# uci-cbcl/RP-Net

Measured on AMD Instinct MI355X. Metric: support/query pairs/sec (fwd+bwd, 1-shot 256x256, T=5), higher is better.
Workload: dtype f32

## Files before the change

rpnet_amd/csrc/conv_split.hip:

```cpp
#include <algorithm>

#include "conv_epilogue.h"
#include "split_bf16.h"

namespace rpnet {

constexpr bool IGLP = true;

template <int NP>
__global__ __launch_bounds__(256) void split_bf16_kernel(const float* __restrict__ x, const float* __restrict__ scale,
                                                          const int mode, unsigned short* __restrict__ out,
                                                          const size_t n8, const FastDiv fC, const size_t plane_elems) {
    RPNET_PASS_PRIORITY();
    for (size_t i = (size_t)blockIdx.x * 256 + threadIdx.x; i < n8; i += (size_t)gridDim.x * 256) {
        const f32x4 a = *reinterpret_cast<const f32x4*>(x + i * 8);
        const f32x4 b = *reinterpret_cast<const f32x4*>(x + i * 8 + 4);
        float v[8] = {a[0], a[1], a[2], a[3], b[0], b[1], b[2], b[3]};
        if (mode) {
            float s = scale[fC.div((unsigned)i)];
            if (mode == 2) s = 1.f - s;
#pragma unroll
            for (int q = 0; q < 8; ++q) v[q] *= s;
        }
        u32x4 o[NP];
        split8<NP>(v, o);
#pragma unroll
        for (int p = 0; p < NP; ++p) *reinterpret_cast<u32x4*>(out + p * plane_elems + i * 8) = o[p];
    }
}

template <int NP>
__global__ __launch_bounds__(256) void split_f16_kernel(const float* __restrict__ x, const float* __restrict__ mask, const int mode,
                                                         const float* __restrict__ s_a, const float* __restrict__ s_b,
                                                         float* __restrict__ s_out, unsigned short* __restrict__ out,
                                                         const size_t n8, const FastDiv fC, const size_t plane_elems,
// ... 137 lines not shown
                if (NP <= 2) {
                    const float inv = 1.f / u_row[row];
#pragma unroll
                    for (int q = 0; q < 8; ++q) v[q] *= inv;
                }
                u32x4 o[NP];
                split8<NP>(v, o);
                const int tf = taps - 1 - tap;
                const size_t dst = (((size_t)tf * (Cout >> 5) + (co0 >> 5)) * Cin_g + row) * 32 + g * 8;
#pragma unroll
                for (int p = 0; p < NP; ++p) *reinterpret_cast<u32x4*>(wd + p * plane + dst) = o[p];
            }
        }
    }
}

__host__ __device__ static inline bool pack_needs_gather(const rpnet_pack_item& q) {
    return (q.cin % 8) || (q.cin_off0 % 8) || (q.cin_split % 8) || (q.cin_off1 % 8);
}

template <int NP>
__global__ __launch_bounds__(256) void pack_weight_split_kernel(const PackItems items) {
    __shared__ float tile[9][32][33];
    const rpnet_pack_item& q = items.it[blockIdx.y];
    const bool gather = pack_needs_gather(q);
    const int tx = gather ? q.cin_pad / 32 : (q.cin + 31) / 32, ntiles = tx * (q.cout / 32);
    if ((int)blockIdx.x >= ntiles) return;
    if (gather)
        pack_weight_split_block<NP, true>(tile, blockIdx.x % tx, blockIdx.x / tx, q.w, (unsigned short*)q.wp, (unsigned short*)q.wd, q.taps,
                                          q.cin_pad, q.cout, q.cin, q.cin_off0, q.cin_split, q.cin_off1, q.row_scale_wp, q.row_scale_wd);
    else
        pack_weight_split_block<NP, false>(tile, blockIdx.x % tx, blockIdx.x / tx, q.w, (unsigned short*)q.wp, (unsigned short*)q.wd, q.taps,
                                           q.cin_pad, q.cout, q.cin, q.cin_off0, q.cin_split, q.cin_off1, q.row_scale_wp, q.row_scale_wd);
}

template <int WGM, int WM, int WN, int NP, bool DB>
__global__ __launch_bounds__(WGM * 128, (DB ? 1 : (WGM == 2 ? 2 : 1))) void conv_igemm_split_kernel(
    const rpnet_conv_desc d, const int M, const int Cin, const int Cout, const int tiles_n, const int ntiles) {
    constexpr int NT = WGM * 128;
    constexpr int BM = 32 * WGM * WM, BN = 64 * WN;
    constexpr int RP = NT / 4;
    constexpr int AJ = BM / RP, BJ = (BN + RP - 1) / RP;
    constexpr bool B_PART = BN < RP;
    constexpr int A_BYTES = BM * 64, B_BYTES = BN * 64;
    constexpr int STAGE = NP * (A_BYTES + B_BYTES);
    __shared__ __attribute__((aligned(16))) unsigned char smem[cmax((DB ? 2 : 1) * STAGE, epilogue_lds_bytes<WN, WGM>())];

    const int t = threadIdx.x;
    const int lane = t & 63, wv = t >> 6;
    const int li = lane & 31, h = lane >> 5;
    const int wm = wv >> 1, wn = wv & 1;

    const int tile = xcd_swizzle(blockIdx.x, ntiles);
    const int tm = tile / tiles_n, tn = tile - tm * tiles_n;
    const int m0 = tm * BM, n0 = tn * BN;

    const int H = d.H, W = d.W, HW = H * W;
    const int ups = d.upsample;
    const int Hs = H >> ups, Ws = W >> ups;
    const int dil = d.dilation > 1 ? d.dilation : 1;

    const int srow = t >> 2, skg = t & 3;
    int rn[AJ], ry[AJ], rx[AJ];
#pragma unroll
    for (int j = 0; j < AJ; ++j) {
        const int m = m0 + srow + RP * j;
// ... 783 lines not shown
    using namespace rpnet;
    RPNET_REQUIRE(items && n >= 1 && n <= kPackMax, RPNET_ERR_ARG, "pack_conv_weights_split: %d items (1..%d)", n, kPackMax);
    RPNET_REQUIRE(planes >= 1 && planes <= 3, RPNET_ERR_SHAPE, "pack_conv_weights_split: planes %d", planes);
    PackItems pk;
    int max_rows = 0, max_tiles = 0;
    for (int i = 0; i < n; ++i) {
        const rpnet_pack_item& q = items[i];
        RPNET_REQUIRE(q.w && q.wp, RPNET_ERR_ARG, "pack_conv_weights_split: null pointer (item %d)", i);
        RPNET_REQUIRE(planes == 3 || (q.row_scale_wp && q.row_scale_wd), RPNET_ERR_ARG,
                      "pack_conv_weights_split: fp16 planes (1 or 2) need the row scale outputs (item %d)", i);
        RPNET_REQUIRE(q.cout > 0 && q.cout % 32 == 0 && q.cin_pad % 32 == 0 && (q.taps == 9 || q.taps == 1 || q.taps == 4), RPNET_ERR_SHAPE,
                      "pack_conv_weights_split: cout %d cin_pad %d taps %d (item %d)", q.cout, q.cin_pad, q.taps, i);
        RPNET_REQUIRE(q.cin > 0 && q.cin_split >= 0 && q.cin_split <= q.cin && q.cin_off0 >= 0 && q.cin_off1 >= 0, RPNET_ERR_SHAPE,
                      "pack_conv_weights_split: cin %d cin_split %d cin_off0 %d cin_off1 %d (item %d)", q.cin, q.cin_split, q.cin_off0,
                      q.cin_off1, i);
        RPNET_REQUIRE((long)q.cin_off0 + q.cin_split <= q.cin_pad && (long)q.cin_off1 + (q.cin - q.cin_split) <= q.cin_pad, RPNET_ERR_SHAPE,
                      "pack_conv_weights_split: channel ranges exceed cin_pad (item %d)", i);
        RPNET_REQUIRE(pack_ranges_disjoint(q.cin, q.cin_off0, q.cin_split, q.cin_off1), RPNET_ERR_SHAPE,
                      "pack_conv_weights_split: channel ranges overlap (item %d)", i);
        pk.it[i] = q;
        max_rows = std::max(max_rows, q.cout + q.cin);
        max_tiles = std::max(max_tiles, (pack_needs_gather(q) ? q.cin_pad / 32 : cdiv(q.cin, 32)) * (q.cout / 32));
    }
    for (int i = n; i < kPackMax; ++i) pk.it[i] = items[0];
    hipStream_t s = (hipStream_t)stream;
    if (planes <= 2)
        hipLaunchKernelGGL(weight_row_scale_kernel, dim3(max_rows, n), dim3(256), 0, s, pk);
    if (planes == 3) hipLaunchKernelGGL(pack_weight_split_kernel<3>, dim3(max_tiles, n), dim3(256), 0, s, pk);
    else if (planes == 2) hipLaunchKernelGGL(pack_weight_split_kernel<2>, dim3(max_tiles, n), dim3(256), 0, s, pk);
    else hipLaunchKernelGGL(pack_weight_split_kernel<1>, dim3(max_tiles, n), dim3(256), 0, s, pk);
    return check_launch("pack_conv_weights_split");
}

extern "C" int rpnet_pack_conv_weight_split(const float* w, void* wp, void* wd, int cout, int cin, int taps, int cin_off0,
                                            int cin_split, int cin_off1, int cin_pad, int planes, float* row_scale_wp,
                                            float* row_scale_wd, rpnet_stream_t stream) {
    rpnet_pack_item q;
    q.w = w; q.wp = wp; q.wd = wd; q.row_scale_wp = row_scale_wp; q.row_scale_wd = row_scale_wd;
    q.cout = cout; q.cin = cin; q.taps = taps; q.cin_off0 = cin_off0; q.cin_split = cin_split; q.cin_off1 = cin_off1; q.cin_pad = cin_pad;
    return rpnet_pack_conv_weights_split(&q, 1, planes, stream);
}
```

rpnet_amd/functional.py:

```python
import collections
import contextlib
import ctypes as C
import os

import torch
from torch.autograd import Function
from torch.autograd.function import once_differentiable

from . import hip
from .hip import ConvDesc, call, ptr, query

BN_EPS = 1e-5
BN_MOMENTUM = 0.1

_ASYNC = {"on": False, "side": {}, "pending": set(), "queued": False, "fifo": [], "keep": []}

_MODES = {"f32": (0, False, 0), "bf16x3": (3, False, 0), "f16x2": (3, True, 2), "f16": (3, True, 1)}
_CORR_PRED_PLANES = True
_MATH = {}


def set_conv_math(mode):
    _MATH["mode"] = mode
    _MATH["planes"], _MATH["f16"], _MATH["f16_planes"] = _MODES[mode]
# ... 474 lines not shown
             self.split, self.off1, self.cin_pad)

    @property
    def wp(self):
        if self._wp is None:
            self._pack_f32()
        return self._wp

    @property
    def wd(self):
        if self._wp is None:
            self._pack_f32()
        return self._wd

    def split_packs(self, planes):
        pk = self.wps.get(planes) if self.wps else None
        if pk is None:
            w = self._weight
            pk = self.alloc_split(planes)
            call("rpnet_pack_conv_weight_split", ptr(w), ptr(pk[0]), ptr(pk[1]), self.cout, self.cin, self.taps,
                 self.off0, self.split, self.off1, self.cin_pad, planes, ptr(pk[2]) if planes <= 2 else None,
                 ptr(pk[3]) if planes <= 2 else None)
        return pk

    def up4_packs(self, planes):
        up = getattr(self, "_up4", None)
        if up is None:
            up = self._up4 = {}
        pk = up.get(planes)
        if pk is None:
            w = self._weight
            wc = torch.empty((4 * self.cout, self.cin, 2, 2), device=w.device, dtype=torch.float32)
            call("rpnet_upconv_collapse_weights", ptr(w), ptr(wc), self.cout, self.cin)
            n = 4 * self.cin * 4 * self.cout
            wp4 = torch.empty((planes, n), device=w.device, dtype=torch.float16)
            wd4 = torch.empty((planes, n), device=w.device, dtype=torch.float16)
            t4 = torch.empty(4 * self.cout, device=w.device, dtype=torch.float32)
            u4 = torch.empty(self.cin, device=w.device, dtype=torch.float32)
            call("rpnet_pack_conv_weight_split", ptr(wc), ptr(wp4), ptr(wd4), 4 * self.cout, self.cin, 4, 0, self.cin, self.cin, self.cin,
                 planes, ptr(t4), ptr(u4))
            pk = up[planes] = (wp4, wd4, t4, u4)
        return pk

    def alloc_split(self, planes):
        if self.wps is None:
            self.wps = {}
        n = self.taps * self.cin_pad * self.cout
        padded = self.cin_pad != self.cin
        w = self._weight
        key = (w.data_ptr(), tuple(w.shape), planes, self.cin_pad, self.off0, self.split, self.off1, str(w.device))
        if padded and self._pool is not None and key in self._pool:
            pk = self._pool[key]
            self.wps[planes] = pk
            return pk
        mk = torch.zeros if padded else torch.empty
        dt = torch.bfloat16 if planes == 3 else torch.float16
        wps, wds = mk((planes, n), device=w.device, dtype=dt), mk((planes, n), device=w.device, dtype=dt)
        if planes == 3:
            pk = (wps, wds)
        else:
            t = torch.empty(self.cout, device=w.device, dtype=torch.float32)
            u = (torch.ones if padded else torch.empty)(self.cin_pad, device=w.device, dtype=torch.float32)
            pk = (wps, wds, t, u)
        if padded and self._pool is not None:
            self._pool[key] = pk
        self.wps[planes] = pk
        return pk


class WeightCache:

    def __init__(self):
        self._d = {}
        self._ready = None
        self._padded = {}

    def clear(self):
        self._d.clear()
        self._ready = None

    def prepack_async(self, weights, planes, device, up4=()):
        main = torch.cuda.current_stream(device)
        ps = _pack_stream(device)
        ps.wait_stream(main)
        self._ready = None
        with torch.cuda.stream(ps):
            self.prepack(weights, planes, up4)
            ev = torch.cuda.Event()
            ev.record(ps)
        self._ready = (ev, set(), torch.cuda.is_current_stream_capturing())

    def get(self, weight, split=None):
        if self._ready is not None and self._ready[2] and not torch.cuda.is_current_stream_capturing():
            self._ready = None
        if self._ready is not None:
            sid = hip.stream()
            if sid not in self._ready[1]:
                torch.cuda.current_stream(weight.device).wait_event(self._ready[0])
                self._ready[1].add(sid)
        key = (weight.data_ptr(), weight._version, None if split is None else tuple(split))
        pw = self._d.get(key)
        if pw is None:
            pw = PackedWeight(weight.detach(), split, self._padded)
            self._d[key] = pw
        return pw

    def prepack(self, weights, planes, up4=()):
        up4 = list(up4) if (_UP4 and planes in (1, 2)) else []
        if up4:
            skip = {id(w) for w in up4}
            weights = [w for w in weights if id(w) not in skip]
            for w in up4:
                self.get(w).up4_packs(planes)
        pws = [self.get(w) for w in weights]
        pws = [pw for pw in pws if pw.taps == 9 and pw.cin_pad == pw.cin and pw.cin % 32 == 0 and pw.cout % 32 == 0
               and not (pw.wps and planes in pw.wps)]
        for i in range(0, len(pws), hip.PACK_MAX):
            chunk = pws[i:i + hip.PACK_MAX]
            items = (hip.PackItem * len(chunk))()
            for it, pw in zip(items, chunk):
                bufs = pw.alloc_split(planes)
                it.w, it.wp, it.wd = ptr(pw._weight), ptr(bufs[0]), ptr(bufs[1])
                it.row_scale_wp, it.row_scale_wd = (ptr(bufs[2]), ptr(bufs[3])) if planes <= 2 else (None, None)
                it.cout, it.cin, it.taps = pw.cout, pw.cin, pw.taps
                it.cin_off0, it.cin_split, it.cin_off1, it.cin_pad = pw.off0, pw.split, pw.off1, pw.cin_pad
            call("rpnet_pack_conv_weights_split", items, len(chunk), planes)

    def materialize(self, weights, planes):
        for w in weights:
            pw = self.get(w)
            if planes and pw.taps == 9 and pw.cin_pad == pw.cin and pw.cin % 32 == 0 and pw.cout % 32 == 0:
                pw.split_packs(planes)
            else:
                pw.wp


TUNE = {"tile": int(os.environ.get("RPNET_TUNE_TILE", "0")) + (0 if os.environ.get("RPNET_CONV_DMA", "1") == "1" else 0x10000),
        "wgrad": int(os.environ.get("RPNET_TUNE_WGRAD", "0"))}


def _desc(x0, x1, w, bias, in_scale, in_mode, y0, y1, N, H, W, taps, ups, groups=1, ep_scale=None, ep_shift=None,
          ep_relu=0, out_scale=None, out_mode=0, accumulate=0, co_split=None, wgrad=False):
    d = ConvDesc()
    d.x0, d.x1 = ptr(x0), ptr(x1)
    d.C0 = x0.shape[-1]
    d.C1 = x1.shape[-1] if x1 is not None else 0
    d.w, d.bias = ptr(w), ptr(bias)
    d.in_scale, d.in_scale_mode = ptr(in_scale), in_mode if in_scale is not None else 0
    d.y0, d.y1 = ptr(y0), ptr(y1)
    d.Co0 = y0.shape[-1] if co_split is None else co_split[0]
    d.Co1 = (y1.shape[-1] if y1 is not None else 0) if co_split is None else co_split[1]
    d.ep_scale, d.ep_shift, d.ep_relu = ptr(ep_scale), ptr(ep_shift), ep_relu
    d.out_scale, d.out_scale_mode, d.accumulate = ptr(out_scale), out_mode if out_scale is not None else 0, accumulate
    d.N, d.H, d.W, d.taps, d.upsample, d.groups = N, H, W, taps, ups, groups
    d.tune = TUNE["wgrad"] if wgrad else TUNE["tile"]
    return d


_Plan = collections.namedtuple("_Plan", "kind planes xs w sx sx1 col", defaults=(None, None, None))


def _conv_plan(pw, op0, op1, in_scale, in_mode, upsample, N, H, W, cout, up4_allowed=True):
    x0, x1 = op0.x, None if op1 is None else op1.x
    if not _use_split(pw, x0, x1):
        return _Plan("f32", 0, (x0, x1), pw.wp)
    f16 = _f16_sources(op0, op1, in_scale, in_mode, pw.taps == 1) if f16_mode() else None
    if f16 is None:
# ... 1065 lines not shown
```

rpnet_amd/hip.py:

```python
import ctypes as C
import os

import torch

_LIB_PATH = os.environ.get("RPNET_LIB_PATH") or os.path.join(os.path.dirname(os.path.abspath(__file__)), "librpnet_hip.so")
_lib = None

vp, ci, cf, cs, cd = C.c_void_p, C.c_int, C.c_float, C.c_size_t, C.c_double


class ConvDesc(C.Structure):
    _fields_ = [("x0", vp), ("x1", vp), ("C0", ci), ("C1", ci), ("w", vp), ("bias", vp), ("in_scale", vp),
                ("in_scale_mode", ci), ("y0", vp), ("y1", vp), ("Co0", ci), ("Co1", ci), ("ep_scale", vp),
                ("ep_shift", vp), ("ep_relu", ci), ("out_scale", vp), ("out_scale_mode", ci), ("accumulate", ci),
                ("N", ci), ("H", ci), ("W", ci), ("taps", ci), ("upsample", ci), ("groups", ci), ("dilation", ci), ("stats_partial", vp), ("split_planes", ci), ("y_split", vp), ("split_out_planes", ci),
                ("acc_scale_col", vp), ("acc_scale_x", vp), ("acc_scale_dy", vp), ("bnb_y", vp), ("bnb_stats", vp), ("bnb_partial", vp), ("bnb_pmax", vp), ("bnb_groups", ci),
                ("acc_scale_x1", vp), ("out_absmax", vp), ("tune", ci), ("y_split_scale", vp), ("splitk_ws", vp), ("splitk_ws_bytes", cs),
                ("skip_mask", vp), ("skip_mode", ci), ("skip_halo", ci), ("skip_ws", vp), ("tile_skip", vp),
                ("y_enc", vp), ("y_enc_stride", ci)]


PACK_MAX = 24


class PackItem(C.Structure):
    _fields_ = [("w", vp), ("wp", vp), ("wd", vp), ("row_scale_wp", vp), ("row_scale_wd", vp), ("cout", ci), ("cin", ci),
                ("taps", ci), ("cin_off0", ci), ("cin_split", ci), ("cin_off1", ci), ("cin_pad", ci)]


_SIGS = {
    "rpnet_version": (ci, []),
    "rpnet_last_error_string": (C.c_char_p, []),
    "rpnet_pack_conv_weight": (ci, [vp, vp, vp, ci, ci, ci, ci, ci, ci, ci, vp]),
    "rpnet_split_bf16": (ci, [vp, vp, ci, vp, cs, ci, ci, vp]),
    "rpnet_split_f16": (ci, [vp, vp, ci, vp, vp, vp, vp, cs, ci, ci, ci, vp]),
    "rpnet_pack_conv_weight_split": (ci, [vp, vp, vp, ci, ci, ci, ci, ci, ci, ci, ci, vp, vp, vp]),
    "rpnet_pack_conv_weights_split": (ci, [C.POINTER(PackItem), ci, ci, vp]),
    "rpnet_conv_fwd": (ci, [C.POINTER(ConvDesc), vp]),
    "rpnet_upconv_collapse_weights": (ci, [vp, vp, ci, ci, vp]),
    "rpnet_conv_up4_supported": (ci, [C.POINTER(ConvDesc), ci]),
    "rpnet_conv_up4_stats_blocks": (ci, [C.POINTER(ConvDesc)]),
    "rpnet_conv_up4": (ci, [C.POINTER(ConvDesc), ci, vp]),
    "rpnet_conv_wgrad_up4_supported": (ci, [C.POINTER(ConvDesc)]),
    "rpnet_conv_wgrad_up4_workspace_bytes": (cs, [ci, ci, ci, ci, ci]),
    "rpnet_conv_wgrad_up4": (ci, [C.POINTER(ConvDesc), vp, vp, vp, cs, vp]),
    "rpnet_conv_stats_blocks": (ci, [C.POINTER(ConvDesc)]),
    "rpnet_conv_tile_variant": (ci, [C.POINTER(ConvDesc)]),
    "rpnet_conv_splitk_workspace_bytes": (cs, [C.POINTER(ConvDesc)]),
    "rpnet_bn_stats_from_partial": (ci, [vp, ci, ci, ci, ci, ci, vp, vp, vp, vp, vp, cf, cf, vp, vp, vp, vp, vp]),
    "rpnet_conv_wgrad_workspace_bytes": (cs, [ci, ci, ci, ci, ci, ci]),
    "rpnet_conv_wgrad": (ci, [C.POINTER(ConvDesc), vp, vp, ci, ci, ci, ci, vp, cs, vp]),
    "rpnet_conv1_fwd": (ci, [vp, vp, vp, vp, vp, vp, ci, ci, ci, ci, vp, vp, ci, vp]),
    "rpnet_conv1_stats_blocks": (ci, [ci, ci, ci, ci, ci]),
    "rpnet_pow2_scale": (ci, [vp, vp, vp]),
    "rpnet_predict_scales": (ci, [vp, vp, vp, ci, cf, ci, vp, vp]),
# ... 204 lines not shown
}
VOLLOAD_ABI_SYMBOLS = tuple(_VOLLOAD_SIGS)
VOLLOAD_ABI_VERSION = 1
SIDE_ABIS_AFTER_SMOOTH = [
    ("rpnet_volload_abi.h", "volume-loading", "rpnet_volload_abi_version", VOLLOAD_ABI_VERSION, _VOLLOAD_SIGS),
]

_DEEDS_SIGS = {
    "rpnet_deeds_abi_version": (ci, []),
    "rpnet_deeds_workspace_bytes": (cs, [ci, ci, ci, ci]),
    "rpnet_deeds_register": (ci, [vp, vp, vp, vp, ci, ci, ci, ci, ci, cf, cf, cf, cf, cf, cf, cf, vp, vp, vp, cs, vp]),
    "rpnet_deeds_warp": (ci, [vp, vp, vp, vp, ci, ci, ci, ci, ci, cf, cf, cf, vp]),
}
DEEDS_ABI_SYMBOLS = tuple(_DEEDS_SIGS)
DEEDS_ABI_VERSION = 1
SIDE_ABIS_AFTER_VOLLOAD = [
    ("rpnet_deeds_abi.h", "DEEDS-registration", "rpnet_deeds_abi_version", DEEDS_ABI_VERSION, _DEEDS_SIGS),
]

_FUSION_RATERS = [C.POINTER(vp), ci, ci, ci, ci, ci, ci]
_FUSION_SIGS = {
    "rpnet_fusion_abi_version": (ci, []),
    "rpnet_fusion_workspace_bytes": (cs, [ci, ci, ci, ci]),
    "rpnet_fusion_patterns": (ci, _FUSION_RATERS + [vp, vp, vp]),
    "rpnet_fusion_fuse": (ci, _FUSION_RATERS + [ci, ci, C.POINTER(cd), ci, ci, cd, vp, ci, vp, vp, ci, vp, C.c_int64, vp, vp, vp, C.c_int64,
                                                C.c_int64, vp, cs, vp]),
}
FUSION_ABI_SYMBOLS = tuple(_FUSION_SIGS)
FUSION_ABI_VERSION = 1
SIDE_ABIS_AFTER_DEEDS = [
    ("rpnet_fusion_abi.h", "label-fusion", "rpnet_fusion_abi_version", FUSION_ABI_VERSION, _FUSION_SIGS),
]


def lib_path():
    return _LIB_PATH


def load():
    global _lib
    if _lib is None:
        if not os.path.exists(_LIB_PATH):
            raise RuntimeError(f"{_LIB_PATH} not found: build it with `make -C rpnet_amd/csrc` "
                               "(or __graft_entry__.build()); rpnet_amd has no CPU fallback")
        lib = C.CDLL(_LIB_PATH)
        lib.rpnet_version.restype = ci
        if lib.rpnet_version() != ABI_VERSION:
            raise RuntimeError(f"{_LIB_PATH} has ABI version {lib.rpnet_version()}, this binding was written for {ABI_VERSION} "
                               "(include/rpnet_abi.h RPNET_ABI_VERSION): rebuild it with `make -C rpnet_amd/csrc`")
        side_abis = (ALL_SIDE_ABIS + SIDE_ABIS_AFTER_PREP + SIDE_ABIS_AFTER_RESAMPLE + SIDE_ABIS_AFTER_SMOOTH + SIDE_ABIS_AFTER_VOLLOAD
                     + SIDE_ABIS_AFTER_DEEDS)
        for sigs in [_SIGS] + [family[4] for family in side_abis]:
            for name, (res, args) in sigs.items():
                fn = getattr(lib, name, None)
                if fn is None:
                    raise RuntimeError(f"{_LIB_PATH} does not export {name}: rebuild it with `make -C rpnet_amd/csrc`")
                fn.restype, fn.argtypes = res, args
        for header, words, version_symbol, version, _ in side_abis:
            if getattr(lib, version_symbol)() != version:
                raise RuntimeError(f"{_LIB_PATH} has {words} ABI version {getattr(lib, version_symbol)()}, this binding was written for "
                                   f"{version} (include/{header}): rebuild it with `make -C rpnet_amd/csrc`")
        _lib = lib
    return _lib


def ptr(t):
    return None if t is None else t.data_ptr()


try:
    _raw_stream, _cur_device = torch._C._cuda_getCurrentRawStream, torch._C._cuda_getDevice
except AttributeError:
    _raw_stream = None


def stream():
    if _raw_stream is not None:
        return _raw_stream(_cur_device())
    return torch.cuda.current_stream().cuda_stream


def call(name, *args):
    lib = load()
    rc = getattr(lib, name)(*args, stream())
# ... 14 lines not shown
```

rpnet_amd/modules.py:

```python
import itertools
import os

import torch
import torch.nn as nn

from . import functional as RF
from .schedule import Schedule

_FANIN = 2
_PREPACK = True
_ZSKIP = True
_F16_MIN_PIXELS = int(os.environ.get("RPNET_F16_MIN_PIXELS", "262144"))
_F16_MIN_PIXELS_EVAL = int(os.environ.get("RPNET_F16_MIN_PIXELS_EVAL", "524288"))
_CRE_STREAMS = True
_CRE_STREAMS_MAX_PIXELS = 16384
_CRE_STREAMS_TRAIN = os.environ.get("RPNET_CRE_STREAMS_TRAIN", "1") == "1"
_ENC_STREAMS = int(os.environ.get("RPNET_ENC_STREAMS", "1"))
_NET_SERIAL = itertools.count(1)


def _to_nhwc(x):
    return x.permute(0, 2, 3, 1).contiguous()


# ... 343 lines not shown
            raise ValueError("n_iter_refinement must be >= 1")
        B = supp_imgs[0][0].shape[0]
        H, W = qry_imgs[0].shape[-2:]
        h, w = H // self.scale, W // self.scale
        cache = self._cache
        RF.reset_async()
        grad_eval = not self.training and torch.is_grad_enabled()
        repack = self.training or not self.freeze_packs or grad_eval or self._packs_from_grad_call
        self._packs_from_grad_call = grad_eval
        if repack:
            cache.clear()

        supp = (supp_imgs[0][0] if n_ways * n_shots == 1 else torch.cat([torch.cat(way, 0) for way in supp_imgs], 0)).float()
        qry = qry_imgs[0].float()
        RF.hip.require_gpu(supp, qry)
        ns = supp.shape[0]
        f16_min, f16_min_eval = sch.get("f16_min_pixels", _F16_MIN_PIXELS), sch.get("f16_min_pixels_eval", _F16_MIN_PIXELS_EVAL)
        thr = f16_min if (self.training or not f16_min_eval or not f16_min or RF._EVAL_PREDICT) else f16_min_eval
        RF.set_f16_active((ns + B) * H * W >= thr)
        pred_key = None
        if RF.f16_mode():
            RF.reset_absmax_pool(supp.device)
            if not self.training and not torch.is_grad_enabled() and RF._EVAL_PREDICT:
                pred_key = (self._serial, RF.conv_math(), ns, B, H, W, self.num_iter, n_ways, n_shots, self.forced_masks is not None)
                RF.pred_begin(supp.device, pred_key, allow=not getattr(self, "_pred_redo", False))
        planes = RF.pack_planes()
        if _PREPACK and planes and repack:
            ups = ()
            if self.training or RF.f16_mode():
                enc_n = (ns + B,) if ns == B else (ns, B)
                ups = tuple(m.up[1].weight for m, f in ((self.encoder.Up5, 8), (self.encoder.Up4, 4))
                            if RF.up4_layer_ok(m.up[1].weight, planes, [(n, H // f, W // f) for n in enc_n + ((ns, B) if ns == B else ())]))
            if self.training and supp.is_cuda:
                cache.prepack_async(self._pack_weights(), planes, supp.device, ups)
            else:
                cache.prepack(self._pack_weights(), planes, ups)
        enc_mask = fore_mask[0][0].float() if self.encoder.mask_feature_map else None
        if enc_mask is not None and ns != B:
            raise NotImplementedError("mask_feature_map with more than one support image per episode: the reference "
                                      "concatenates B masks onto Wa*Sh*B images (net/unet.py:438) and fails")
        enc_streams, fanin = sch.get("enc_streams", _ENC_STREAMS), sch.get("fanin", _FANIN)
        two_chains = (self.training and supp.is_cuda and enc_mask is None and
                      (enc_streams == 2 or (enc_streams == 1 and ns != B and ns <= 2 * B)))
        RF.order_begin(two_chains)
        split_fan = False
        if ns == B and not two_chains:
            d4 = self.encoder.forward_nhwc(torch.cat([supp, qry], 0).reshape(ns + B, H, W, 1), cache, groups=2,
                                           mask=None if enc_mask is None else torch.cat([enc_mask, enc_mask], 0))
            s_supp = s_qry = d4.scale
            d4 = d4.x
            split_fan = d4.requires_grad and fanin >= 2 and n_ways * n_shots == 1
            if split_fan:
                uses = RF.SplitFan.apply(d4, ns, 2, 2 * self.num_iter)
                supp_d4, qry_d4, fan_supp, fan_qry = uses[0], uses[2], uses[:2], uses[2:]
            else:
                supp_d4, qry_d4 = RF.SplitRows.apply(d4, ns) if (d4.requires_grad and fanin) else (d4[:ns], d4[ns:])
        elif two_chains:
            main, side = torch.cuda.current_stream(supp.device), RF._cre_stream(supp.device)
            qin = qry.reshape(B, H, W, 1)
            cache.materialize([w for w in self._pack_weights() if w is not self.cre.w_k[0].weight and w is not self.cre.w_q[0].weight],
                              planes)
            side.wait_stream(main)
            o_s = self.encoder.forward_nhwc(supp.reshape(ns, H, W, 1), cache)
            with torch.cuda.stream(side):
                o_q = self.encoder.forward_nhwc(qin, cache)
            qin.record_stream(side)
            main.wait_stream(side)
# ... 145 lines not shown
```

Baseline: 497.8.

## Fuse per-step weight packing into one multi-item kernel with staged readiness events

Replaces the chunked per-layer weight packing (row-scale kernel plus pack kernel per chunk of 24, separate upconv collapse) with one fused packer. A tile-max pass reduces row and column absmax into a scratch workspace with atomics, and a single pack kernel then emits the split planes for up to 48 layers, collapsing the upconv 3x3 into 2x2 phases in place. Prepacking is also split into an early group (the first encoder convs) and the rest, each with its own event, so the first encoder layers can start before every weight is packed. The cost is an extra memset and a workspace allocation each step, plus more complex synchronisation bookkeeping.

```diff
diff --git a/include/rpnet_pack_fused_abi.h b/include/rpnet_pack_fused_abi.h
--- /dev/null
+++ b/include/rpnet_pack_fused_abi.h
@@ -0,0 +1,26 @@
+#ifndef RPNET_PACK_FUSED_ABI_H
+#define RPNET_PACK_FUSED_ABI_H
+
+#include <stddef.h>
+#include <stdint.h>
+
+#include "rpnet_abi.h"
+
+#ifdef __cplusplus
+extern "C" {
+#endif
+
+#define RPNET_PACK_FUSED_ABI_VERSION 1
+int rpnet_pack_fused_abi_version(void);
+
+#define RPNET_PACK_FUSED_MAX 48
+
+size_t rpnet_pack_conv_weights_fused_workspace_bytes(const rpnet_pack_item* items, const int* collapse, int n, int planes);
+int rpnet_pack_conv_weights_fused(const rpnet_pack_item* items, const int* collapse, int n, int planes, void* workspace,
+                                  size_t workspace_bytes, rpnet_stream_t stream);
+
+#ifdef __cplusplus
+}
+#endif
+
+#endif
diff --git a/rpnet_amd/csrc/conv_split.hip b/rpnet_amd/csrc/conv_split.hip
--- a/rpnet_amd/csrc/conv_split.hip
+++ b/rpnet_amd/csrc/conv_split.hip
@@ -1,6 +1,7 @@
 #include <algorithm>
 
 #include "conv_epilogue.h"
+#include "rpnet_pack_fused_abi.h"
 #include "split_bf16.h"
 
 namespace rpnet {
@@ -204,6 +205,232 @@
     else
         pack_weight_split_block<NP, false>(tile, blockIdx.x % tx, blockIdx.x / tx, q.w, (unsigned short*)q.wp, (unsigned short*)q.wd, q.taps,
                                            q.cin_pad, q.cout, q.cin, q.cin_off0, q.cin_split, q.cin_off1, q.row_scale_wp, q.row_scale_wd);
+}
+
+constexpr int kFusedMax = RPNET_PACK_FUSED_MAX;
+struct FusedItem {
+    const float* w; unsigned short* wp; unsigned short* wd; float* t; float* u;
+    int cout, cin, taps, off0, split, off1;
+    int collapse, tile0, scr0;
+    int vec;
+};
+struct FusedItems {
+    FusedItem it[kFusedMax];
+    unsigned* scratch;
+    int n;
+};
+static_assert(sizeof(FusedItems) <= 4096 - 64, "the item table is a kernel argument");
+
+struct FusedTile { int item, ci0, by, ncin; };
+
+__device__ __forceinline__ FusedTile fused_find_tile(const FusedItems& items) {
+    int i = 0;
+    while (i + 1 < items.n && (int)blockIdx.x >= items.it[i + 1].tile0) ++i;
+    const FusedItem& q = items.it[i];
+    const int tile = (int)blockIdx.x - q.tile0, tx = (q.cin + 31) >> 5;
+    const int by = tile / tx, bx = tile - by * tx;
+    return FusedTile{i, bx * 32, by, min(32, q.cin - bx * 32)};
+}
+
+__device__ __forceinline__ void fused_load_tile(float (*tile)[32][33], const float* __restrict__ w, const int taps, const int cin_w,
+                                                const int ci0, const int co0, const int ncin, const bool vec) {
+    const int nel = ncin * taps;
+    const unsigned inv = (65536u + taps - 1) / taps;
+    if (vec) {
+        const int nq = nel >> 2;
+        const unsigned mq = (1u << 20) / nq + 1;
+        const float* const base = w + ((size_t)co0 * cin_w + ci0) * taps;
+        const size_t run = (size_t)cin_w * taps;
+        f32x4 v[9];
+#pragma unroll
+        for (int j = 0; j < 9; ++j) {
+            const int f = (int)threadIdx.x + 256 * j, col = (int)(((unsigned)f * mq) >> 20);
+            if (col < 32) v[j] = *reinterpret_cast<const f32x4*>(base + col * run + 4 * (f - col * nq));
+        }
+#pragma unroll
+        for (int j = 0; j < 9; ++j) {
+            const int f = (int)threadIdx.x + 256 * j, col = (int)(((unsigned)f * mq) >> 20);
+            if (col < 32) {
+#pragma unroll
+                for (int i = 0; i < 4; ++i) {
+                    const int r = 4 * (f - col * nq) + i, c = (int)(((unsigned)r * inv) >> 16);
+                    tile[r - c * taps][c][col] = v[j][i];
+                }
+            }
+        }
+        return;
+    }
+    int col = (int)threadIdx.x / nel, r = (int)threadIdx.x - col * nel;
+    while (col < 32) {
+        const int c = (int)(((unsigned)r * inv) >> 16), tap = r - c * taps;
+        tile[tap][c][col] = w[((size_t)(co0 + col) * cin_w + ci0) * taps + r];
+        r += 256;
+        while (r >= nel) { r -= nel; ++col; }
+    }
+}
+
+__device__ __forceinline__ void fused_take_taps(float (*tile)[32][33], const int ncin, float (&k)[4][9]) {
+#pragma unroll
+    for (int j = 0; j < 4; ++j) {
+        const int p = (int)threadIdx.x + 256 * j, col = p & 31, c = p >> 5;
+#pragma unroll
+        for (int q = 0; q < 9; ++q) k[j][q] = c < ncin ? tile[q][c][col] : 0.f;
+    }
+}
+
+template <int PY, int PX>
+__device__ __forceinline__ void fused_put_phase(float (*tile)[32][33], const int ncin, const float (&k)[4][9]) {
+#pragma unroll
+    for (int j = 0; j < 4; ++j) {
+        const int p = (int)threadIdx.x + 256 * j, col = p & 31, cl = p >> 5;
+        if (cl >= ncin) continue;
+#pragma unroll
+        for (int r = 0; r < 2; ++r)
+#pragma unroll
+            for (int c = 0; c < 2; ++c) {
+                constexpr int y1 = PY ? 2 : 1, y0e = PY ? 1 : 0, x1 = PX ? 2 : 1, x0e = PX ? 1 : 0;
+                const int ya = r == 0 ? 0 : y1, yb = r == 0 ? y0e : 2;
+                const int xa = c == 0 ? 0 : x1, xb = c == 0 ? x0e : 2;
+                float s = 0.f;
+#pragma unroll
+                for (int ky = 0; ky < 3; ++ky)
+#pragma unroll
+                    for (int kx = 0; kx < 3; ++kx)
+                        if (ky >= ya && ky <= yb && kx >= xa && kx <= xb) s += k[j][ky * 3 + kx];
+                tile[r * 2 + c][cl][col] = s;
+            }
+    }
+}
+
+__device__ __forceinline__ void fused_tile_maxima(float (*tile)[32][33], float (*red)[4][32], const int taps, const int ncin,
+                                                  unsigned* __restrict__ scr_t, unsigned* __restrict__ scr_u) {
+    const int t = threadIdx.x, which = t >> 7, idx = t & 31, part = (t >> 5) & 3;
+    float m = 0.f;
+    if (which == 0) {
+        const int c1 = min(part * 8 + 8, ncin);
+        for (int tap = 0; tap < taps; ++tap)
+            for (int c = part * 8; c < c1; ++c) m = fmaxf(m, fabsf(tile[tap][c][idx]));
+    } else if (idx < ncin) {
+        for (int tap = 0; tap < taps; ++tap)
+#pragma unroll
+            for (int col = part * 8; col < part * 8 + 8; ++col) m = fmaxf(m, fabsf(tile[tap][idx][col]));
+    }
+    red[which][part][idx] = m;
+    __syncthreads();
+    if (t < 64) {
+        const int wh = t >> 5;
+        m = fmaxf(fmaxf(red[wh][0][idx], red[wh][1][idx]), fmaxf(red[wh][2][idx], red[wh][3][idx]));
+        if (m > 0.f && (wh == 0 || idx < ncin)) atomicMax((wh == 0 ? scr_t : scr_u) + idx, __float_as_uint(m));
+    }
+}
+
+__global__ __launch_bounds__(256) void weight_tile_max_kernel(const FusedItems items) {
+    __shared__ float tile[9][32][33];
+    __shared__ float red[2][4][32];
+    const FusedTile ft = fused_find_tile(items);
+    const FusedItem& q = items.it[ft.item];
+    unsigned* const scr = items.scratch + q.scr0;
+    fused_load_tile(tile, q.w, q.taps, q.cin, ft.ci0, ft.by * 32, ft.ncin, q.vec != 0);
+    __syncthreads();
+    if (!q.collapse) {
+        fused_tile_maxima(tile, red, q.taps, ft.ncin, scr + ft.by * 32, scr + q.cout + ft.ci0);
+        return;
+    }
+    float k[4][9];
+    fused_take_taps(tile, ft.ncin, k);
+    unsigned* const scr_u = scr + 4 * q.cout + ft.ci0;
+#define RPNET_FUSED_PHASE(PY, PX)                                                                              \
+    __syncthreads();                                                                                           \
+    fused_put_phase<PY, PX>(tile, ft.ncin, k);                                                                 \
+    __syncthreads();                                                                                           \
+    fused_tile_maxima(tile, red, 4, ft.ncin, scr + ((PY) * 2 + (PX)) * q.cout + ft.by * 32, scr_u);
+    RPNET_FUSED_PHASE(0, 0) RPNET_FUSED_PHASE(0, 1) RPNET_FUSED_PHASE(1, 0) RPNET_FUSED_PHASE(1, 1)
+#undef RPNET_FUSED_PHASE
+}
+
+template <int NP>
+__device__ __forceinline__ void fused_emit(float (*tile)[32][33], const int ci0, const int co0, const int ncin, unsigned short* __restrict__ wp,
+                                           unsigned short* __restrict__ wd, const int taps, const int Cin_g, const int Cout, const int off0,
+                                           const int split, const int off1, const unsigned* __restrict__ scr_t,
+                                           const unsigned* __restrict__ scr_u, float* __restrict__ t_out, float* __restrict__ u_out,
+                                           const bool pub_t, const bool pub_u) {
+    const int t = threadIdx.x;
+    if (NP <= 2) {
+        if (pub_t && t < 32) t_out[co0 + t] = pow2_scale(__uint_as_float(scr_t[co0 + t]));
+        if (pub_u && t >= 64 && t < 64 + ncin) {
+            const int cin = ci0 + t - 64;
+            u_out[cin < split ? off0 + cin : off1 + (cin - split)] = pow2_scale(__uint_as_float(scr_u[cin]));
+        }
+    }
+    const size_t plane = (size_t)taps * Cin_g * Cout;
+    for (int e = t; e < taps * 32 * 4; e += 256) {
+        const int g = e & 3, cl = (e >> 2) & 31, tap = e >> 7;
+        if (g * 8 < ncin) {
+            const int cin = ci0 + g * 8;
+            const int row = cin < split ? off0 + cin : off1 + (cin - split);
+            float v[8];
+#pragma unroll
+            for (int q = 0; q < 8; ++q) v[q] = tile[tap][g * 8 + q][cl];
+            if (NP <= 2) {
+                const float inv = 1.f / pow2_scale(__uint_as_float(scr_t[co0 + cl]));
+#pragma unroll
+                for (int q = 0; q < 8; ++q) v[q] *= inv;
+            }
+            u32x4 o[NP];
+            split8<NP>(v, o);
+            const size_t dst = (((size_t)tap * (Cin_g >> 5) + (row >> 5)) * Cout + co0 + cl) * 32 + (row & 31);
+#pragma unroll
+            for (int p = 0; p < NP; ++p) *reinterpret_cast<u32x4*>(wp + p * plane + dst) = o[p];
+        }
+    }
+    if (wd) {
+        for (int e = t; e < taps * 32 * 4; e += 256) {
+            const int g = e & 3, c = (e >> 2) & 31, tap = e >> 7;
+            if (c < ncin) {
+                const int cin = ci0 + c;
+                const int row = cin < split ? off0 + cin : off1 + (cin - split);
+                float v[8];
+#pragma unroll
+                for (int q = 0; q < 8; ++q) v[q] = tile[tap][c][g * 8 + q];
+                if (NP <= 2) {
+                    const float inv = 1.f / pow2_scale(__uint_as_float(scr_u[cin]));
+#pragma unroll
+                    for (int q = 0; q < 8; ++q) v[q] *= inv;
+                }
+                u32x4 o[NP];
+                split8<NP>(v, o);
+                const int tf = taps - 1 - tap;
+                const size_t dst = (((size_t)tf * (Cout >> 5) + (co0 >> 5)) * Cin_g + row) * 32 + g * 8;
+#pragma unroll
+                for (int p = 0; p < NP; ++p) *reinterpret_cast<u32x4*>(wd + p * plane + dst) = o[p];
+            }
+        }
+    }
+}
+
+template <int NP>
+__global__ __launch_bounds__(256) void pack_weight_fused_kernel(const FusedItems items) {
+    __shared__ float tile[9][32][33];
+    const FusedTile ft = fused_find_tile(items);
+    const FusedItem& q = items.it[ft.item];
+    const unsigned* const scr = items.scratch + q.scr0;
+    fused_load_tile(tile, q.w, q.taps, q.cin, ft.ci0, ft.by * 32, ft.ncin, q.vec != 0);
+    __syncthreads();
+    if (!q.collapse) {
+        fused_emit<NP>(tile, ft.ci0, ft.by * 32, ft.ncin, q.wp, q.wd, q.taps, q.cin, q.cout, q.off0, q.split, q.off1, scr, scr + q.cout, q.t,
+                       q.u, ft.ci0 == 0, ft.by == 0);
+        return;
+    }
+    float k[4][9];
+    fused_take_taps(tile, ft.ncin, k);
+#define RPNET_FUSED_PHASE(PY, PX)                                                                                                  \
+    __syncthreads();                                                                                                               \
+    fused_put_phase<PY, PX>(tile, ft.ncin, k);                                                                                     \
+    __syncthreads();                                                                                                               \
+    fused_emit<NP>(tile, ft.ci0, ((PY) * 2 + (PX)) * q.cout + ft.by * 32, ft.ncin, q.wp, q.wd, 4, q.cin, 4 * q.cout, q.off0, q.split,  \
+                   q.off1, scr, scr + 4 * q.cout, q.t, q.u, ft.ci0 == 0, ft.by == 0 && (PY) * 2 + (PX) == 0);
+    RPNET_FUSED_PHASE(0, 0) RPNET_FUSED_PHASE(0, 1) RPNET_FUSED_PHASE(1, 0) RPNET_FUSED_PHASE(1, 1)
+#undef RPNET_FUSED_PHASE
 }
 
 template <int WGM, int WM, int WN, int NP, bool DB>
@@ -1053,6 +1280,83 @@
     return check_launch("pack_conv_weights_split");
 }
 
+namespace rpnet {
+
+static int fused_plan(const rpnet_pack_item* items, const int* collapse, int n, int planes, FusedItems* pk, int* tiles, size_t* words) {
+    RPNET_REQUIRE(items && n >= 1 && n <= kFusedMax, RPNET_ERR_ARG, "pack_conv_weights_fused: %d items (1..%d)", n, kFusedMax);
+    RPNET_REQUIRE(planes >= 1 && planes <= 3, RPNET_ERR_SHAPE, "pack_conv_weights_fused: planes %d", planes);
+    long nt = 0, nw = 0;
+    for (int i = 0; i < n; ++i) {
+        const rpnet_pack_item& q = items[i];
+        const int up = collapse && collapse[i];
+        RPNET_REQUIRE(q.w && q.wp, RPNET_ERR_ARG, "pack_conv_weights_fused: null pointer (item %d)", i);
+        RPNET_REQUIRE(planes == 3 || (q.row_scale_wp && q.row_scale_wd), RPNET_ERR_ARG,
+                      "pack_conv_weights_fused: fp16 planes (1 or 2) need the row scale outputs (item %d)", i);
+        RPNET_REQUIRE(q.cout > 0 && q.cout % 32 == 0 && q.cin_pad % 32 == 0 && (q.taps == 9 || q.taps == 1 || q.taps == 4), RPNET_ERR_SHAPE,
+                      "pack_conv_weights_fused: cout %d cin_pad %d taps %d (item %d)", q.cout, q.cin_pad, q.taps, i);
+        RPNET_REQUIRE(q.cin > 0 && q.cin_split >= 0 && q.cin_split <= q.cin && q.cin_off0 >= 0 && q.cin_off1 >= 0, RPNET_ERR_SHAPE,
+                      "pack_conv_weights_fused: cin %d cin_split %d cin_off0 %d cin_off1 %d (item %d)", q.cin, q.cin_split, q.cin_off0,
+                      q.cin_off1, i);
+        RPNET_REQUIRE((long)q.cin_off0 + q.cin_split <= q.cin_pad && (long)q.cin_off1 + (q.cin - q.cin_split) <= q.cin_pad, RPNET_ERR_SHAPE,
+                      "pack_conv_weights_fused: channel ranges exceed cin_pad (item %d)", i);
+        RPNET_REQUIRE(pack_ranges_disjoint(q.cin, q.cin_off0, q.cin_split, q.cin_off1), RPNET_ERR_SHAPE,
+                      "pack_conv_weights_fused: channel ranges overlap (item %d)", i);
+        RPNET_REQUIRE(!pack_needs_gather(q) && q.cin_pad == q.cin, RPNET_ERR_SHAPE,
+                      "pack_conv_weights_fused: a gathered or padded layer (cin %d cin_pad %d) takes rpnet_pack_conv_weights_split (item %d)",
+                      q.cin, q.cin_pad, i);
+        RPNET_REQUIRE(!up || (q.taps == 9 && q.cin_off0 == 0 && q.cin_split == q.cin), RPNET_ERR_SHAPE,
+                      "pack_conv_weights_fused: a collapsed layer is a plain 3x3 layer (item %d)", i);
+        FusedItem& f = pk->it[i];
+        f.w = q.w; f.wp = (unsigned short*)q.wp; f.wd = (unsigned short*)q.wd; f.t = q.row_scale_wp; f.u = q.row_scale_wd;
+        f.cout = q.cout; f.cin = q.cin; f.taps = q.taps; f.off0 = q.cin_off0; f.split = q.cin_split; f.off1 = q.cin_off1;
+        f.collapse = up; f.tile0 = (int)nt; f.scr0 = (int)nw; f.vec = ((uintptr_t)q.w & 15) == 0;
+        nt += (long)cdiv(q.cin, 32) * (q.cout / 32);
+        nw += (long)(up ? 4 : 1) * q.cout + q.cin;
+        RPNET_REQUIRE(nt < (1l << 30) && nw < (1l << 30), RPNET_ERR_SHAPE, "pack_conv_weights_fused: too many tiles (item %d)", i);
+    }
+    for (int i = n; i < kFusedMax; ++i) pk->it[i] = pk->it[0];
+    pk->n = n;
+    pk->scratch = nullptr;
+    *tiles = (int)nt;
+    *words = planes <= 2 ? (size_t)nw : 0;
+    return RPNET_OK;
+}
+
+}
+
+extern "C" int rpnet_pack_fused_abi_version(void) { return RPNET_PACK_FUSED_ABI_VERSION; }
+
+extern "C" size_t rpnet_pack_conv_weights_fused_workspace_bytes(const rpnet_pack_item* items, const int* collapse, int n, int planes) {
+    rpnet::FusedItems pk;
+    int tiles = 0;
+    size_t words = 0;
+    if (rpnet::fused_plan(items, collapse, n, planes, &pk, &tiles, &words) != RPNET_OK) return 0;
+    return words * sizeof(unsigned);
+}
+
+extern "C" int rpnet_pack_conv_weights_fused(const rpnet_pack_item* items, const int* collapse, int n, int planes, void* workspace,
+                                             size_t workspace_bytes, rpnet_stream_t stream) {
+    using namespace rpnet;
+    FusedItems pk;
+    int tiles = 0;
+    size_t words = 0;
+    const int rc = fused_plan(items, collapse, n, planes, &pk, &tiles, &words);
+    if (rc != RPNET_OK) return rc;
+    hipStream_t s = (hipStream_t)stream;
+    if (planes <= 2) {
+        RPNET_REQUIRE(workspace && workspace_bytes >= words * sizeof(unsigned) && ((uintptr_t)workspace & 3) == 0, RPNET_ERR_WORKSPACE,
+                      "pack_conv_weights_fused: workspace of %zu bytes, %zu needed", workspace_bytes, words * sizeof(unsigned));
+        pk.scratch = (unsigned*)workspace;
+        const hipError_t e = hipMemsetAsync(workspace, 0, words * sizeof(unsigned), s);
+        RPNET_REQUIRE(e == hipSuccess, (int)e, "pack_conv_weights_fused: hipMemsetAsync: %s", hipGetErrorString(e));
+        hipLaunchKernelGGL(weight_tile_max_kernel, dim3(tiles), dim3(256), 0, s, pk);
+    }
+    if (planes == 3) hipLaunchKernelGGL(pack_weight_fused_kernel<3>, dim3(tiles), dim3(256), 0, s, pk);
+    else if (planes == 2) hipLaunchKernelGGL(pack_weight_fused_kernel<2>, dim3(tiles), dim3(256), 0, s, pk);
+    else hipLaunchKernelGGL(pack_weight_fused_kernel<1>, dim3(tiles), dim3(256), 0, s, pk);
+    return check_launch("pack_conv_weights_fused");
+}
+
 extern "C" int rpnet_pack_conv_weight_split(const float* w, void* wp, void* wd, int cout, int cin, int taps, int cin_off0,
                                             int cin_split, int cin_off1, int cin_pad, int planes, float* row_scale_wp,
                                             float* row_scale_wd, rpnet_stream_t stream) {
diff --git a/rpnet_amd/functional.py b/rpnet_amd/functional.py
--- a/rpnet_amd/functional.py
+++ b/rpnet_amd/functional.py
@@ -530,14 +530,21 @@
             w = self._weight
             wc = torch.empty((4 * self.cout, self.cin, 2, 2), device=w.device, dtype=torch.float32)
             call("rpnet_upconv_collapse_weights", ptr(w), ptr(wc), self.cout, self.cin)
-            n = 4 * self.cin * 4 * self.cout
-            wp4 = torch.empty((planes, n), device=w.device, dtype=torch.float16)
-            wd4 = torch.empty((planes, n), device=w.device, dtype=torch.float16)
-            t4 = torch.empty(4 * self.cout, device=w.device, dtype=torch.float32)
-            u4 = torch.empty(self.cin, device=w.device, dtype=torch.float32)
-            call("rpnet_pack_conv_weight_split", ptr(wc), ptr(wp4), ptr(wd4), 4 * self.cout, self.cin, 4, 0, self.cin, self.cin, self.cin,
-                 planes, ptr(t4), ptr(u4))
-            pk = up[planes] = (wp4, wd4, t4, u4)
+            pk = self.alloc_up4(planes)
+            call("rpnet_pack_conv_weight_split", ptr(wc), ptr(pk[0]), ptr(pk[1]), 4 * self.cout, self.cin, 4, 0, self.cin, self.cin, self.cin,
+                 planes, ptr(pk[2]), ptr(pk[3]))
+        return pk
+
+    def alloc_up4(self, planes):
+        up = getattr(self, "_up4", None)
+        if up is None:
+            up = self._up4 = {}
+        w, n = self._weight, 4 * self.cin * 4 * self.cout
+        wp4 = torch.empty((planes, n), device=w.device, dtype=torch.float16)
+        wd4 = torch.empty((planes, n), device=w.device, dtype=torch.float16)
+        t4 = torch.empty(4 * self.cout, device=w.device, dtype=torch.float32)
+        u4 = torch.empty(self.cin, device=w.device, dtype=torch.float32)
+        pk = up[planes] = (wp4, wd4, t4, u4)
         return pk
 
     def alloc_split(self, planes):
@@ -571,31 +578,49 @@
     def __init__(self):
         self._d = {}
         self._ready = None
+        self._group = {}
+        self._ws = []
         self._padded = {}
 
     def clear(self):
         self._d.clear()
         self._ready = None
-
-    def prepack_async(self, weights, planes, device, up4=()):
+        self._group = {}
+        self._ws = []
+
+    def prepack_async(self, weights, planes, device, up4=(), early=()):
         main = torch.cuda.current_stream(device)
         ps = _pack_stream(device)
         ps.wait_stream(main)
         self._ready = None
+        first = {id(w) for w in early}
+        groups = [g for g in ([w for w in weights if id(w) in first], [w for w in weights if id(w) not in first]) if g]
+        capturing = torch.cuda.is_current_stream_capturing()
+        ready, self._group = [], {}
         with torch.cuda.stream(ps):
-            self.prepack(weights, planes, up4)
-            ev = torch.cuda.Event()
-            ev.record(ps)
-        self._ready = (ev, set(), torch.cuda.is_current_stream_capturing())
+            for g, ws in enumerate(groups):
+                last = g == len(groups) - 1
+                here = {id(w) for w in ws}
+                self.prepack(ws, planes, [w for w in up4 if id(w) in here or last])
+                ev = torch.cuda.Event()
+                ev.record(ps)
+                ready.append([ev, set(), capturing])
+                for w in ws:
+                    self._group[w.data_ptr()] = g
+            for w in up4:
+                self._group.setdefault(w.data_ptr(), len(groups) - 1)
+        self._ready = ready or None
 
     def get(self, weight, split=None):
-        if self._ready is not None and self._ready[2] and not torch.cuda.is_current_stream_capturing():
+        if self._ready is not None and self._ready[0][2] and not torch.cuda.is_current_stream_capturing():
             self._ready = None
         if self._ready is not None:
             sid = hip.stream()
-            if sid not in self._ready[1]:
-                torch.cuda.current_stream(weight.device).wait_event(self._ready[0])
-                self._ready[1].add(sid)
+            g = self._group.get(weight.data_ptr())
+            for r in (self._ready if g is None else self._ready[g:g + 1]):
+                if sid not in r[1]:
+                    torch.cuda.current_stream(weight.device).wait_event(r[0])
+                    r[1].add(sid)
         key = (weight.data_ptr(), weight._version, None if split is None else tuple(split))
         pw = self._d.get(key)
         if pw is None:
@@ -605,16 +630,40 @@
 
     def prepack(self, weights, planes, up4=()):
         up4 = list(up4) if (_UP4 and planes in (1, 2)) else []
-        if up4:
-            skip = {id(w) for w in up4}
-            weights = [w for w in weights if id(w) not in skip]
-            for w in up4:
-                self.get(w).up4_packs(planes)
-        pws = [self.get(w) for w in weights]
+        skip = {id(w) for w in up4}
+        pws = [self.get(w) for w in weights if id(w) not in skip]
         pws = [pw for pw in pws if pw.taps == 9 and pw.cin_pad == pw.cin and pw.cin % 32 == 0 and pw.cout % 32 == 0
                and not (pw.wps and planes in pw.wps)]
-        for i in range(0, len(pws), hip.PACK_MAX):
-            chunk = pws[i:i + hip.PACK_MAX]
+        ups = [pw for pw in (self.get(w) for w in up4) if planes not in (getattr(pw, "_up4", None) or {})]
+        n = len(pws) + len(ups)
+        if n == 0:
+            return
+        items, flags = (hip.PackItem * n)(), (C.c_int * n)()
+        for i, pw in enumerate(pws + ups):
+            up = i >= len(pws)
+            bufs = pw.alloc_up4(planes) if up else pw.alloc_split(planes)
+            it = items[i]
+            it.w, it.wp, it.wd = ptr(pw._weight), ptr(bufs[0]), ptr(bufs[1])
+            it.row_scale_wp, it.row_scale_wd = (ptr(bufs[2]), ptr(bufs[3])) if planes <= 2 else (None, None)
+            it.cout, it.cin, it.taps = pw.cout, pw.cin, pw.taps
+            it.cin_off0, it.cin_split, it.cin_off1, it.cin_pad = pw.off0, pw.split, pw.off1, pw.cin_pad
+            flags[i] = int(up)
+        nbytes = query("rpnet_pack_conv_weights_fused_workspace_bytes", items, flags, n, planes)
+        ws = torch.empty(max(nbytes, 16), device=pws[0]._weight.device if pws else ups[0]._weight.device, dtype=torch.uint8)
+        self._ws.append(ws)
+        call("rpnet_pack_conv_weights_fused", items, flags, n, planes, ptr(ws), nbytes)
+
+    def materialize(self, weights, planes):
+        missing = []
+        for w in weights:
+            pw = self.get(w)
+            if planes and pw.taps == 9 and pw.cin_pad == pw.cin and pw.cin % 32 == 0 and pw.cout % 32 == 0:
+                if not (pw.wps and planes in pw.wps) and not any(pw is m for m in missing):
+                    missing.append(pw)
+            else:
+                pw.wp
+        for i in range(0, len(missing), hip.PACK_MAX):
+            chunk = missing[i:i + hip.PACK_MAX]
             items = (hip.PackItem * len(chunk))()
             for it, pw in zip(items, chunk):
                 bufs = pw.alloc_split(planes)
@@ -623,14 +672,6 @@
                 it.cout, it.cin, it.taps = pw.cout, pw.cin, pw.taps
                 it.cin_off0, it.cin_split, it.cin_off1, it.cin_pad = pw.off0, pw.split, pw.off1, pw.cin_pad
             call("rpnet_pack_conv_weights_split", items, len(chunk), planes)
-
-    def materialize(self, weights, planes):
-        for w in weights:
-            pw = self.get(w)
-            if planes and pw.taps == 9 and pw.cin_pad == pw.cin and pw.cin % 32 == 0 and pw.cout % 32 == 0:
-                pw.split_packs(planes)
-            else:
-                pw.wp
 
 
 TUNE = {"tile": int(os.environ.get("RPNET_TUNE_TILE", "0")) + (0 if os.environ.get("RPNET_CONV_DMA", "1") == "1" else 0x10000),
diff --git a/rpnet_amd/hip.py b/rpnet_amd/hip.py
--- a/rpnet_amd/hip.py
+++ b/rpnet_amd/hip.py
@@ -21,6 +21,7 @@
 
 
 PACK_MAX = 24
+FUSED_MAX = 48
 
 
 class PackItem(C.Structure):
@@ -291,6 +292,17 @@
     ("rpnet_fusion_abi.h", "label-fusion", "rpnet_fusion_abi_version", FUSION_ABI_VERSION, _FUSION_SIGS),
 ]
 
+_PACK_FUSED_SIGS = {
+    "rpnet_pack_fused_abi_version": (ci, []),
+    "rpnet_pack_conv_weights_fused_workspace_bytes": (cs, [C.POINTER(PackItem), C.POINTER(ci), ci, ci]),
+    "rpnet_pack_conv_weights_fused": (ci, [C.POINTER(PackItem), C.POINTER(ci), ci, ci, vp, cs, vp]),
+}
+PACK_FUSED_ABI_SYMBOLS = tuple(_PACK_FUSED_SIGS)
+PACK_FUSED_ABI_VERSION = 1
+SIDE_ABIS_AFTER_FUSION = [
+    ("rpnet_pack_fused_abi.h", "fused-packer", "rpnet_pack_fused_abi_version", PACK_FUSED_ABI_VERSION, _PACK_FUSED_SIGS),
+]
+
 
 def lib_path():
     return _LIB_PATH
@@ -308,7 +320,7 @@
             raise RuntimeError(f"{_LIB_PATH} has ABI version {lib.rpnet_version()}, this binding was written for {ABI_VERSION} "
                                "(include/rpnet_abi.h RPNET_ABI_VERSION): rebuild it with `make -C rpnet_amd/csrc`")
         side_abis = (ALL_SIDE_ABIS + SIDE_ABIS_AFTER_PREP + SIDE_ABIS_AFTER_RESAMPLE + SIDE_ABIS_AFTER_SMOOTH + SIDE_ABIS_AFTER_VOLLOAD
-                     + SIDE_ABIS_AFTER_DEEDS)
+                     + SIDE_ABIS_AFTER_DEEDS + SIDE_ABIS_AFTER_FUSION)
         for sigs in [_SIGS] + [family[4] for family in side_abis]:
             for name, (res, args) in sigs.items():
                 fn = getattr(lib, name, None)
diff --git a/rpnet_amd/modules.py b/rpnet_amd/modules.py
--- a/rpnet_amd/modules.py
+++ b/rpnet_amd/modules.py
@@ -399,7 +399,9 @@
                 ups = tuple(m.up[1].weight for m, f in ((self.encoder.Up5, 8), (self.encoder.Up4, 4))
                             if RF.up4_layer_ok(m.up[1].weight, planes, [(n, H // f, W // f) for n in enc_n + ((ns, B) if ns == B else ())]))
             if self.training and supp.is_cuda:
-                cache.prepack_async(self._pack_weights(), planes, supp.device, ups)
+                enc = self.encoder
+                early = [m.weight for m in (enc.Conv1.conv[0], enc.Conv1.conv[3], enc.Conv2.conv[0], enc.Conv2.conv[3])]
+                cache.prepack_async(self._pack_weights(), planes, supp.device, ups, early)
             else:
                 cache.prepack(self._pack_weights(), planes, ups)
         enc_mask = fore_mask[0][0].float() if self.encoder.mask_feature_map else None
```

Result: no change. 502.5, median of 6 (+1.0%).
